# ai4ce/DiscoNet

Measured on AMD Instinct MI355X. Metric: scenes/sec (5-agent 256x256 BEV), higher is better.
Workload: dtype f16 hi+lo pair per value (32 bits; 22-bit significand for |x| >= 0.125, f16 exponent range, lo subnormal below: absolute floor 2^-25); conv products as split-f16 x3 MFMA, f32 accumulate; 1 GPU; DiscoNet det eval forward (--com disco), 5-agent, batch 4 per GPU, 256x256x13 BEV, no KD, sparse voxel lists -> dense -> enc -> DiscoGraph fusion -> dec -> cls/reg heads; agents=5, batch_per_gpu=4, conv_math=sp, launch=hipGraph replay, parallelism=scene-parallel x1 (no data-path collective)

## Files before the change

disconet_amd/csrc/common.hip:

```cpp
#include "dn_internal.h"

namespace dn {
char* err_buf() {
  static thread_local char buf[512] = {0};
  return buf;
}
namespace {
typedef unsigned u32x4 __attribute__((ext_vector_type(4)));
__global__ void __launch_bounds__(256) zero_fill_kernel(unsigned char* p, size_t head, size_t vecs, size_t tail) {
  const size_t tid = blockIdx.x * (size_t)blockDim.x + threadIdx.x, stride = (size_t)gridDim.x * blockDim.x;
  if (tid < head) p[tid] = 0;
  u32x4* v = reinterpret_cast<u32x4*>(p + head);
  for (size_t i = tid; i < vecs; i += stride) v[i] = u32x4{0u, 0u, 0u, 0u};
  if (tid < tail) p[head + 16 * vecs + tid] = 0;
}
}

hipError_t zero_fill(void* ptr, size_t bytes, hipStream_t stream) {
  if (bytes == 0) return hipSuccess;
  unsigned char* p = static_cast<unsigned char*>(ptr);
  size_t head = (16 - (reinterpret_cast<size_t>(p) & 15)) & 15;
  if (head > bytes) head = bytes;
  const size_t vecs = (bytes - head) / 16, tail = bytes - head - 16 * vecs;
  const size_t want = (vecs + 255) / 256;
  const int blocks = (int)(want < 1 ? 1 : (want > 8192 ? 8192 : want));
  hipLaunchKernelGGL(zero_fill_kernel, dim3(blocks), dim3(256), 0, stream, p, head, vecs, tail);
  return hipGetLastError();
}
}

extern "C" int dn_version(void) { return 135; }

#ifndef DN_BUILD_ID
#error "build through disconet_amd/csrc/build.py (it passes -DDN_BUILD_ID)"
#endif
static const char dn_build_id_marker[] = "dn-build-id:" DN_BUILD_ID;
extern "C" const char* dn_build_id(void) { return dn_build_id_marker + 12; }

extern "C" int dn_sp_range_flags_async(unsigned* dst_device, int reset, void* stream) {
  DN_REQUIRE(dst_device != nullptr, "sp_range_flags_async: null destination");
  hipStream_t s = (hipStream_t)stream;
  if ((reset & 2) && dn::zero_fill(dst_device, sizeof(unsigned), s) != hipSuccess)
    return dn::fail(DN_ERR_LAUNCH, "sp_range_flags_async: zero fill of the destination failed");
  const bool clear = (reset & 1) != 0;
  dn::range_collect_conv_sp(dst_device, clear, s);
  dn::range_collect_conv_spq(dst_device, clear, s);
  dn::range_collect_fuse_mlp(dst_device, clear, s);
  dn::range_collect_conv_wgrad(dst_device, clear, s);
  return dn::check_launch("sp_range_collect_kernel");
}

extern "C" unsigned dn_sp_range_flags(int reset) {
  unsigned* d = nullptr;
  unsigned v = 0;
  if (hipDeviceSynchronize() != hipSuccess || hipMalloc((void**)&d, sizeof v) != hipSuccess) return 0x80000000u;
  bool ok = hipMemcpy(d, &v, sizeof v, hipMemcpyHostToDevice) == hipSuccess &&
            dn_sp_range_flags_async(d, reset ? 1 : 0, nullptr) == DN_OK &&
            hipMemcpy(&v, d, sizeof v, hipMemcpyDeviceToHost) == hipSuccess;
  (void)hipFree(d);
  return ok ? v : 0x80000000u;
}

extern "C" const char* dn_last_error(void) { return dn::err_buf(); }
```

disconet_amd/csrc/fuse_mlp.hip:

```cpp
#include "dn_internal.h"
#include "sp_device.h"
#include <type_traits>

#ifndef DN_FUSE_PHASES
#define DN_FUSE_PHASES 0
#endif
#if DN_FUSE_PHASES
__device__ unsigned long long g_fuse_phase[8];
extern "C" int dn_fuse_phase_cycles(unsigned long long* host8, int reset) {
  if (hipDeviceSynchronize() != hipSuccess) return -1;
  if (host8 && hipMemcpyFromSymbol(host8, HIP_SYMBOL(g_fuse_phase), sizeof(unsigned long long) * 8) != hipSuccess) return -1;
  if (reset) { unsigned long long z[8] = {0}; if (hipMemcpyToSymbol(HIP_SYMBOL(g_fuse_phase), z, sizeof z) != hipSuccess) return -1; }
  return 0;
}
#endif

namespace {

constexpr int MAX_AGENTS = 8;
constexpr size_t kW2Bytes = 8 * 2 * 2 * 32 * 16, kW3Bytes = 2 * 2 * 2 * 32 * 16;
constexpr int FUSE_G = 3;
constexpr int FUSE_GL = 2;

struct FuseMlpArgs {
  const float* feat;
  const float* warped;
  const int32_t* num_agent;
  const unsigned char* w1;
  const unsigned char* w2;
  const unsigned char* w3;
  const float *s1, *t1, *s2, *t2, *s3, *t3, *w4, *b4;
  unsigned char* fused_sp;
  float* fused_nhwc;
  float* weights_out;
  int batch, agents, hw, only_v2i, ego_first, ego_count, tiles;
  int total_tiles;
  int warped_fm;
};
constexpr int kWAhead = 1, kWRing = 2;

__device__ inline half8 frag_of(const unsigned char* base, int idx) {
  return *reinterpret_cast<const half8*>(base + (size_t)idx * 16);
}

template <int C, int G, int NW, int WL = 0>
__global__ void __launch_bounds__(64 * (WL > 0 ? WL : NW), (NW == 1 || WL > 0) ? 1 : 2) disco_fuse_mlp_kernel(const FuseMlpArgs a) {
  constexpr bool kWL = WL > 0;
  constexpr int TWV = kWL ? WL : 1;
  static_assert(!kWL || NW == 1, "weight-in-LDS form: one wave per tile");
  constexpr int KS = C / 16;
  constexpr int KSW = KS / NW;
  static_assert(KS % NW == 0, "pass 2 splits the k-steps over the waves");
  constexpr int kW1MatBytes = 4 * KS * 2 * 2 * 32 * 16;
  extern __shared__ __attribute__((aligned(16))) unsigned char w1_s[];
  __shared__ float ek_s[TWV][MAX_AGENTS][64];
  __shared__ float e_s[kWL ? 1 : 64][64];
  __shared__ int jl_s[TWV][MAX_AGENTS];
  __shared__ __attribute__((aligned(16))) unsigned char w23_s[kW2Bytes + kW3Bytes];
  __shared__ __attribute__((aligned(16))) float aff_s[2 * 128 + 2 * 32 + 3 * 8];

  const int lane = threadIdx.x & 63, wave = NW > 1 ? threadIdx.x >> 6 : 0;
  const int tw = kWL ? threadIdx.x >> 6 : 0;
  const int ks_first = wave * KSW;
  const int li = lane & 31, lh = lane >> 5;
  const int wid_raw = kWL ? blockIdx.x * WL + tw : blockIdx.x;
  const bool have = wid_raw < a.total_tiles;
  const int wid = have ? wid_raw : a.total_tiles - 1;
  const int tile = wid % a.tiles, il = (wid / a.tiles) % a.ego_count, b = wid / (a.tiles * a.ego_count);
  const int i = a.ego_first + il;
  const int p = tile * 32 + li;
  const bool pvalid = p < a.hw && have;
  const int pc = p < a.hw ? p : a.hw - 1;
  int live = a.num_agent[b];
  live = live < 0 ? 0 : (live < a.agents ? live : a.agents);
  const size_t oimg = (size_t)il * a.batch + b;

  struct Row {
    const float* p;
    int kss, r1;
  };
  const Row xrow_r = {a.feat + (((size_t)i * a.batch + b) * a.hw + pc) * C + 8 * lh, 16, 4};
  const float* xrow = xrow_r.p;
  auto yrow_of = [&](int j) {
    const int jj = j - (j > i ? 1 : 0);
    const float* pair = a.warped + (((size_t)b * a.ego_count + il) * (a.agents - 1) + jj) * a.hw * C;
    return a.warped_fm ? Row{pair + ((size_t)tile * KS * 2 * 64 + lane) * 4, 512, 256} : Row{pair + (size_t)pc * C + 8 * lh, 16, 4};
  };

  float amax = 0.f;
  bool nan_seen = false;
  auto store_piece = [&](int ks, const f32x4 v0, const f32x4 v1) {
    if (!pvalid) return;
    if (a.fused_sp) {
      u32x2 h0, l0, h1, l1;
      note_nan4(nan_seen, v0);
      note_nan4(nan_seen, v1);
      split4(v0, h0, l0, amax);
      split4(v1, h1, l1, amax);
      const size_t plane = (size_t)a.hw * 16;
      unsigned char* o = a.fused_sp + ((oimg * KS + ks) * 4 + lh) * plane + (size_t)p * 16;
      *reinterpret_cast<u32x4*>(o) = u32x4{h0[0], h0[1], h1[0], h1[1]};
      *reinterpret_cast<u32x4*>(o + 2 * plane) = u32x4{l0[0], l0[1], l1[0], l1[1]};
    }
    if (a.fused_nhwc) {
      float* o = a.fused_nhwc + (oimg * a.hw + p) * C + 16 * ks + 8 * lh;
      *reinterpret_cast<f32x4*>(o) = v0;
      *reinterpret_cast<f32x4*>(o + 4) = v1;
    }
  };

  constexpr int NTHR = 64 * (kWL ? WL : NW);
#if DN_FUSE_PHASES
  unsigned long long ph[8] = {0, 0, 0, 0, 0, 0, 0, 0};
  unsigned long long t_prev = __builtin_readcyclecounter();
  const unsigned long long t_begin = t_prev;
  auto mark = [&](int k) { const unsigned long long t = __builtin_readcyclecounter(); ph[k] += t - t_prev; t_prev = t; };
#else
  auto mark = [&](int) {};
#endif
  if (kWL || i < live) {
    const int t = threadIdx.x;
    for (int q = t; q < (int)((kW2Bytes + kW3Bytes) / 16); q += NTHR)
      *reinterpret_cast<u32x4*>(w23_s + q * 16) = *reinterpret_cast<const u32x4*>(a.w2 + (size_t)q * 16);
    for (int q = t; q < 128; q += NTHR) { aff_s[q] = a.s1[q]; aff_s[128 + q] = a.t1[q]; }
    if (t < 32) { aff_s[256 + t] = a.s2[t]; aff_s[288 + t] = a.t2[t]; }
    if (t < 8) { aff_s[320 + t] = a.s3[t]; aff_s[328 + t] = a.t3[t]; aff_s[336 + t] = a.w4[t]; }
  }
  auto stage_w1 = [&](int mat) {
    if constexpr (kWL) {
      const auto rs = __builtin_amdgcn_make_buffer_rsrc(const_cast<unsigned char*>(a.w1 + (size_t)mat * kW1MatBytes), 0,
                                                        kW1MatBytes, 0x00020000);
      constexpr int INSTR = kW1MatBytes / 1024;
      for (int q = tw; q < INSTR; q += WL) dma16(rs, w1_s + q * 1024, (unsigned)(q * 1024 + lane * 16), 0);
      wait_vm0();
    }
  };
  stage_w1(0);
  const float b4v = a.b4[0];
  const unsigned char* w2l = w23_s;
  const unsigned char* w3l = w23_s + kW2Bytes;
  const float *s1l = aff_s, *t1l = aff_s + 128, *s2l = aff_s + 256, *t2l = aff_s + 288, *s3l = aff_s + 320,
              *t3l = aff_s + 328, *w4l = aff_s + 336;

  const bool active = have && i < live;
  if (i >= live) {
#pragma unroll
    for (int u = 0; u < KSW; ++u) {
      const int ks = ks_first + u;
      store_piece(ks, *reinterpret_cast<const f32x4*>(xrow + 16 * ks),
                  *reinterpret_cast<const f32x4*>(xrow + 16 * ks + 4));
    }
    if constexpr (!kWL) {
      note_range(amax, nan_seen);
      return;
    }
  }

  int n = 1;
  jl_s[tw][0] = i;
  for (int j = 0; j < live; ++j)
    if (j != i && (!a.only_v2i || i == 0 || j == 0)) jl_s[tw][n++] = j;
  if constexpr (NW > 1 || kWL) __syncthreads();
  auto row_of = [&](int k) { return k == 0 ? xrow_r : yrow_of(jl_s[tw][k]); };

  auto frag_from = [&](const f32x4 v0, const f32x4 v1, half8& fh, half8& fl) {
    u32x2 h0, l0, h1, l1;
    split4(v0, h0, l0);
    split4(v1, h1, l1);
    fh = __builtin_bit_cast(half8, u32x4{h0[0], h0[1], h1[0], h1[1]});
    fl = __builtin_bit_cast(half8, u32x4{l0[0], l0[1], l1[0], l1[1]});
  };

  auto layer1 = [&](auto ng_c, const Row (&rows)[G], int cnt, int mat, f32x16 (&acc)[G][4]) {
    constexpr int NG = decltype(ng_c)::value;
    const unsigned char* wbase = a.w1 + (size_t)mat * 4 * KS * 2 * 2 * 32 * 16 + (size_t)(lh * 32 + li) * 16;
    half8 wh[kWRing][4], wl[kWRing][4];
    constexpr int RING = 4;
    f32x4 r0[RING][NG], r1[RING][NG];
    auto wload = [&](int ks, int s) {
#pragma unroll
      for (int nt = 0; nt < 4; ++nt) {
        if constexpr (kWL) {
          wh[s][nt] = *reinterpret_cast<const half8*>(w1_s + (((nt * KS + ks) * 2 + 0) * 64 + lh * 32 + li) * 16);
          wl[s][nt] = *reinterpret_cast<const half8*>(w1_s + (((nt * KS + ks) * 2 + 1) * 64 + lh * 32 + li) * 16);
        } else {
          wh[s][nt] = *reinterpret_cast<const half8*>(wbase + (size_t)(((nt * KS + ks) * 2 + 0) * 64) * 16);
          wl[s][nt] = *reinterpret_cast<const half8*>(wbase + (size_t)(((nt * KS + ks) * 2 + 1) * 64) * 16);
        }
      }
    };
    auto rload = [&](int ks, int s) {
#pragma unroll
      for (int g = 0; g < NG; ++g)
        if (g < cnt) {
          r0[s][g] = *reinterpret_cast<const f32x4*>(rows[g].p + ks * rows[g].kss);
          r1[s][g] = *reinterpret_cast<const f32x4*>(rows[g].p + ks * rows[g].kss + rows[g].r1);
        }
    };
    auto mma = [&](int sw, int sr) {
#pragma unroll
      for (int g = 0; g < NG; ++g)
        if (g < cnt) {
          half8 fh, fl;
          frag_from(r0[sr][g], r1[sr][g], fh, fl);
#pragma unroll
          for (int nt = 0; nt < 4; ++nt) acc[g][nt] = __builtin_amdgcn_mfma_f32_32x32x16_f16(wl[sw][nt], fh, acc[g][nt], 0, 0, 0);
#pragma unroll
          for (int nt = 0; nt < 4; ++nt) acc[g][nt] = __builtin_amdgcn_mfma_f32_32x32x16_f16(wh[sw][nt], fl, acc[g][nt], 0, 0, 0);
#pragma unroll
          for (int nt = 0; nt < 4; ++nt) acc[g][nt] = __builtin_amdgcn_mfma_f32_32x32x16_f16(wh[sw][nt], fh, acc[g][nt], 0, 0, 0);
        }
    };
    static_assert(KS % RING == 0, "k loop runs RING k-steps per trip");
#pragma unroll
    for (int q = 0; q < RING - 1; ++q) rload(q, q);
#pragma unroll
    for (int q = 0; q < kWAhead; ++q) wload(q, q);
#pragma unroll 1
    for (int ks0 = 0; ks0 < KS; ks0 += RING) {
#pragma unroll
      for (int u = 0; u < RING; ++u) {
        const int ks = ks0 + u;
        if (ks + RING - 1 < KS) rload(ks + RING - 1, (u + RING - 1) % RING);
        if (ks + kWAhead < KS) wload(ks + kWAhead, (u + kWAhead) & (kWRing - 1));
        __builtin_amdgcn_sched_barrier(0);
        mma(u & (kWRing - 1), u);
        __builtin_amdgcn_sched_barrier(0);
      }
    }
  };

  auto tail = [&](f32x16 (&acc)[4]) -> float {
    f32x16 acc2;
#pragma unroll
    for (int r = 0; r < 16; ++r) acc2[r] = 0.f;
#pragma unroll
    for (int nt = 0; nt < 4; ++nt) {
      u32x2 hi[4], lo[4];
#pragma unroll
      for (int g = 0; g < 4; ++g) {
        const int u = nt * 32 + 8 * g + 4 * lh;
        const f32x4 sc = *reinterpret_cast<const f32x4*>(s1l + u), sh = *reinterpret_cast<const f32x4*>(t1l + u);
        float unused = 0.f;
        split4(affine4(quad_of(acc[nt], g), sc, sh), hi[g], lo[g], unused, 0.f);
      }
#pragma unroll
      for (int m = 0; m < 2; ++m) {
        const int ks = nt * 2 + m;
        const half8 xh = __builtin_bit_cast(half8, gather_octet(hi[2 * m], hi[2 * m + 1]));
        const half8 xl = __builtin_bit_cast(half8, gather_octet(lo[2 * m], lo[2 * m + 1]));
        const half8 wh = frag_of(w2l, ((ks * 2 + 0) * 2 + lh) * 32 + li), wl = frag_of(w2l, ((ks * 2 + 1) * 2 + lh) * 32 + li);
        acc2 = __builtin_amdgcn_mfma_f32_32x32x16_f16(wl, xh, acc2, 0, 0, 0);
        acc2 = __builtin_amdgcn_mfma_f32_32x32x16_f16(wh, xl, acc2, 0, 0, 0);
        acc2 = __builtin_amdgcn_mfma_f32_32x32x16_f16(wh, xh, acc2, 0, 0, 0);
      }
    }
    f32x16 acc3;
#pragma unroll
    for (int r = 0; r < 16; ++r) acc3[r] = 0.f;
    {
      u32x2 hi[4], lo[4];
#pragma unroll
      for (int g = 0; g < 4; ++g) {
        const int u = 8 * g + 4 * lh;
        const f32x4 sc = *reinterpret_cast<const f32x4*>(s2l + u), sh = *reinterpret_cast<const f32x4*>(t2l + u);
        float unused = 0.f;
        split4(affine4(quad_of(acc2, g), sc, sh), hi[g], lo[g], unused, 0.f);
      }
#pragma unroll
      for (int m = 0; m < 2; ++m) {
        const half8 xh = __builtin_bit_cast(half8, gather_octet(hi[2 * m], hi[2 * m + 1]));
        const half8 xl = __builtin_bit_cast(half8, gather_octet(lo[2 * m], lo[2 * m + 1]));
        const half8 wh = frag_of(w3l, ((m * 2 + 0) * 2 + lh) * 32 + li), wl = frag_of(w3l, ((m * 2 + 1) * 2 + lh) * 32 + li);
        acc3 = __builtin_amdgcn_mfma_f32_32x32x16_f16(wl, xh, acc3, 0, 0, 0);
        acc3 = __builtin_amdgcn_mfma_f32_32x32x16_f16(wh, xl, acc3, 0, 0, 0);
        acc3 = __builtin_amdgcn_mfma_f32_32x32x16_f16(wh, xh, acc3, 0, 0, 0);
      }
    }
    const f32x4 sc = *reinterpret_cast<const f32x4*>(s3l + 4 * lh), sh = *reinterpret_cast<const f32x4*>(t3l + 4 * lh);
    const f32x4 w4 = *reinterpret_cast<const f32x4*>(w4l + 4 * lh);
    float part = 0.f;
#pragma unroll
    for (int e = 0; e < 4; ++e) part += fmaxf(acc3[e] * sc[e] + sh[e], 0.f) * w4[e];
    const float other = __shfl_xor(part, 32, 64);
    const float s = fmaxf((lh ? other + part : part + other) + b4v, 0.f);
    return expf(s);
  };

  f32x16 Ereg[kWL ? 4 : 1];
  mark(0);
  if constexpr (kWL) {
    if (active) {
      f32x16 acc[G][4];
#pragma unroll
      for (int nt = 0; nt < 4; ++nt)
#pragma unroll
        for (int r = 0; r < 16; ++r) acc[0][nt][r] = 0.f;
      Row rows[G];
#pragma unroll
      for (int g = 0; g < G; ++g) rows[g] = xrow_r;
      layer1(std::integral_constant<int, 1>{}, rows, 1, 0, acc);
#pragma unroll
      for (int nt = 0; nt < 4; ++nt) Ereg[nt] = acc[0][nt];
#if DN_FUSE_PHASES
      { float probe = Ereg[0][0]; asm volatile("v_mov_b32 %0, %0" : "+v"(probe)); }
#endif
    }
    mark(1);
    __syncthreads();
    stage_w1(1);
    __syncthreads();
    mark(0);
  } else if constexpr (NW == 1) {
    f32x16 acc[G][4];
#pragma unroll
    for (int nt = 0; nt < 4; ++nt)
#pragma unroll
      for (int r = 0; r < 16; ++r) acc[0][nt][r] = 0.f;
    Row rows[G];
#pragma unroll
    for (int g = 0; g < G; ++g) rows[g] = xrow_r;
    layer1(std::integral_constant<int, 1>{}, rows, 1, 0, acc);
#pragma unroll
    for (int nt = 0; nt < 4; ++nt)
#pragma unroll
      for (int r = 0; r < 16; ++r) e_s[nt * 16 + r][lane] = acc[0][nt][r];
  } else {
    static_assert(NW == 1 || NW == 4, "one layer-1 unit tile per wave");
    f32x16 acc;
#pragma unroll
    for (int r = 0; r < 16; ++r) acc[r] = 0.f;
    const unsigned char* wb = a.w1 + (size_t)(lh * 32 + li) * 16 + (size_t)(wave * KS) * 2 * 64 * 16;
    half8 wh[2], wl[2];
    f32x4 r0[4], r1[4];
    auto wload = [&](int ks, int sl) {
      wh[sl] = *reinterpret_cast<const half8*>(wb + (size_t)((ks * 2 + 0) * 64) * 16);
      wl[sl] = *reinterpret_cast<const half8*>(wb + (size_t)((ks * 2 + 1) * 64) * 16);
    };
    auto rload = [&](int ks, int sl) {
      r0[sl] = *reinterpret_cast<const f32x4*>(xrow + 16 * ks);
      r1[sl] = *reinterpret_cast<const f32x4*>(xrow + 16 * ks + 4);
    };
    rload(0, 0);
    rload(1, 1);
    rload(2, 2);
    wload(0, 0);
#pragma unroll 1
    for (int ks0 = 0; ks0 < KS; ks0 += 4) {
#pragma unroll
      for (int u = 0; u < 4; ++u) {
        const int ks = ks0 + u;
        if (ks + 3 < KS) rload(ks + 3, (u + 3) & 3);
        if (ks + 1 < KS) wload(ks + 1, (u + 1) & 1);
        half8 fh, fl;
        frag_from(r0[u], r1[u], fh, fl);
        acc = __builtin_amdgcn_mfma_f32_32x32x16_f16(wl[u & 1], fh, acc, 0, 0, 0);
        acc = __builtin_amdgcn_mfma_f32_32x32x16_f16(wh[u & 1], fl, acc, 0, 0, 0);
        acc = __builtin_amdgcn_mfma_f32_32x32x16_f16(wh[u & 1], fh, acc, 0, 0, 0);
      }
    }
#pragma unroll
    for (int r = 0; r < 16; ++r) e_s[wave * 16 + r][lane] = acc[r];
    __syncthreads();
  }
  if constexpr (kWL) {
    if (!active) {
      note_range(amax, nan_seen);
      return;
    }
  }
  if constexpr (NW == 1) {
    for (int g0 = 0; g0 < n; g0 += G) {
      const int cnt = n - g0 < G ? n - g0 : G;
      f32x16 acc[G][4];
      Row rows[G];
#pragma unroll
      for (int g = 0; g < G; ++g) {
        rows[g] = row_of(g0 + g < n ? g0 + g : 0);
        if (g < cnt) {
#pragma unroll
          for (int nt = 0; nt < 4; ++nt) {
            if constexpr (kWL) acc[g][nt] = Ereg[nt];
            else {
#pragma unroll
              for (int r = 0; r < 16; ++r) acc[g][nt][r] = e_s[nt * 16 + r][lane];
            }
          }
        }
      }
      layer1(std::integral_constant<int, G>{}, rows, cnt, 1, acc);
#if DN_FUSE_PHASES
      { float probe = acc[0][0][0]; asm volatile("v_mov_b32 %0, %0" : "+v"(probe)); }
#endif
      mark(2);
#pragma unroll
      for (int g = 0; g < G; ++g)
        if (g < cnt) ek_s[tw][g0 + g][lane] = tail(acc[g]);
      mark(3);
    }
  } else {
    for (int k = wave; k < n; k += NW) {
      f32x16 acc[G][4];
      Row rows[G];
#pragma unroll
      for (int g = 0; g < G; ++g) rows[g] = row_of(k);
#pragma unroll
      for (int nt = 0; nt < 4; ++nt)
#pragma unroll
        for (int r = 0; r < 16; ++r) acc[0][nt][r] = e_s[nt * 16 + r][lane];
      layer1(std::integral_constant<int, 1>{}, rows, 1, 1, acc);
      ek_s[0][k][lane] = tail(acc[0]);
    }
    __syncthreads();
  }
  float den = 0.f;
  for (int k = 0; k < n; ++k) den += ek_s[tw][k][lane];

  f32x4 f0[KSW], f1[KSW], y0[2][KSW], y1[2][KSW];
  auto yload = [&](int k, int s) {
    const Row row = row_of(k);
#pragma unroll
    for (int ks = 0; ks < KSW; ++ks) {
      y0[s][ks] = *reinterpret_cast<const f32x4*>(row.p + (ks_first + ks) * row.kss);
      y1[s][ks] = *reinterpret_cast<const f32x4*>(row.p + (ks_first + ks) * row.kss + row.r1);
    }
  };
  auto yacc = [&](int k, int s) {
    const float w = ek_s[tw][k][lane] / den;
    if (a.weights_out && pvalid && lh == 0 && wave == 0)
      a.weights_out[(((size_t)b * a.ego_count + il) * a.agents + k) * a.hw + p] = w;
#pragma unroll
    for (int ks = 0; ks < KSW; ++ks) {
      f0[ks] += y0[s][ks] * w;
      f1[ks] += y1[s][ks] * w;
    }
  };
#pragma unroll
  for (int ks = 0; ks < KSW; ++ks) f0[ks] = f1[ks] = f32x4{0.f, 0.f, 0.f, 0.f};
  yload(0, 0);
  for (int k = 0; k < n; k += 2) {
    if (k + 1 < n) yload(k + 1, 1);
    yacc(k, 0);
    if (k + 1 < n) {
      if (k + 2 < n) yload(k + 2, 0);
      yacc(k + 1, 1);
    }
  }
#pragma unroll
  for (int ks = 0; ks < KSW; ++ks) store_piece(ks_first + ks, f0[ks], f1[ks]);
  note_range(amax, nan_seen);
#if DN_FUSE_PHASES
  mark(4);
  ph[5] = 1;
  ph[6] = __builtin_readcyclecounter() - t_begin;
  if (lane == 0)
    for (int k = 0; k < 7; ++k) atomicAdd(&g_fuse_phase[k], ph[k]);
#endif
}

__global__ void pack_frags_kernel(const float* __restrict__ w, int ld, int col0, int rows, int cols,
                                  int n_tiles, int ksteps, float wmul, unsigned char* __restrict__ out) {
  const int idx = blockIdx.x * blockDim.x + threadIdx.x;
  if (idx >= n_tiles * ksteps * 2 * 32) return;
  const int row = idx % 32, h = (idx / 32) % 2, ks = (idx / 64) % ksteps, nt = idx / (64 * ksteps);
  half8 hi, lo;
#pragma unroll
  for (int e = 0; e < 8; ++e) {
    const int r = nt * 32 + row, c = ks * 16 + h * 8 + e;
    float v = (r < rows && c < cols) ? w[(size_t)r * ld + col0 + c] * wmul : 0.f;
    v = fminf(fmaxf(v, -65504.f), 65504.f);
    hi[e] = (_Float16)v;
    lo[e] = (_Float16)(v - (float)hi[e]);
  }
  *reinterpret_cast<half8*>(out + (size_t)((((nt * ksteps + ks) * 2 + 0) * 2 + h) * 32 + row) * 16) = hi;
  *reinterpret_cast<half8*>(out + (size_t)((((nt * ksteps + ks) * 2 + 1) * 2 + h) * 32 + row) * 16) = lo;
}

inline size_t w1_bytes(int c) { return (size_t)2 * 4 * (c / 16) * 2 * 2 * 32 * 16; }

}

namespace dn { void range_collect_fuse_mlp(unsigned* dst, bool reset, hipStream_t s) { sp_range_collect_here(dst, reset, s); } }

int g_fuse_waves = 0;

extern "C" int dn_fuse_mlp_set_waves(int waves) {
  DN_REQUIRE(waves == 0 || waves == 1 || waves == 2 || waves == 4,
             "fuse_mlp: form is 1 or 4 waves per tile, 2 = layer-1 weights in LDS (0 = default), got %d", waves);
  g_fuse_waves = waves;
  return DN_OK;
}

extern "C" int dn_fuse_mlp_supported(int c) { return c == 64 || c == 128 || c == 256; }

extern "C" size_t dn_fuse_mlp_packed_bytes(int c) { return w1_bytes(c) + kW2Bytes + kW3Bytes; }

extern "C" int dn_fuse_mlp_pack(const float* w1, const float* w2, const float* w3, int c, float wmul1,
                                float wmul2, float wmul3, void* packed, void* stream) {
  DN_REQUIRE(w1 && w2 && w3 && packed, "fuse_mlp pack: null pointer");
  DN_REQUIRE(dn_fuse_mlp_supported(c), "fuse_mlp pack: %d channels unsupported (64, 128 or 256)", c);
  hipStream_t s = (hipStream_t)stream;
  unsigned char* out = (unsigned char*)packed;
  const int ks = c / 16;
  for (int mat = 0; mat < 2; ++mat)
    hipLaunchKernelGGL(pack_frags_kernel, dim3((4 * ks * 64 + 255) / 256), dim3(256), 0, s, w1, 2 * c, mat * c,
                       128, c, 4, ks, wmul1, out + (size_t)mat * (w1_bytes(c) / 2));
  hipLaunchKernelGGL(pack_frags_kernel, dim3((8 * 64 + 255) / 256), dim3(256), 0, s, w2, 128, 0, 32, 128, 1, 8,
                     wmul2, out + w1_bytes(c));
  hipLaunchKernelGGL(pack_frags_kernel, dim3((2 * 64 + 255) / 256), dim3(256), 0, s, w3, 32, 0, 8, 32, 1, 2,
                     wmul3, out + w1_bytes(c) + kW2Bytes);
  return dn::check_launch("pack_frags_kernel");
}

namespace {
template <int CC, int WL>
int launch_wl(const FuseMlpArgs& a, dim3 grid, int lds, hipStream_t s) {
  auto kern = disco_fuse_mlp_kernel<CC, FUSE_GL, 1, WL>;
  static dn::PerDeviceFlag flag;
  bool& done = flag.here();
  if (!done) {
    if (hipFuncSetAttribute(reinterpret_cast<const void*>(kern), hipFuncAttributeMaxDynamicSharedMemorySize, lds) != hipSuccess)
      return dn::fail(DN_ERR_LAUNCH, "fuse_mlp: cannot reserve %d B of dynamic LDS", lds);
    done = true;
  }
  hipLaunchKernelGGL(kern, grid, dim3(64 * WL), lds, s, a);
  return dn::check_launch("disco_fuse_mlp_kernel (weights in LDS)");
}

int fuse_mlp_impl(const float* feat, const float* warped, int warped_fm, const int32_t* num_agent, const dn_fuse_mlp_params* p,
                  int batch, int agents, int hw, int c, int only_v2i, int ego_first, int ego_count, void* fused_sp,
                  float* fused_nhwc, float* weights_out, void* stream);
}

extern "C" int dn_disco_fuse_mlp(const float* feat, const float* warped, const int32_t* num_agent,
                                 const dn_fuse_mlp_params* p, int batch, int agents, int hw, int c,
                                 int only_v2i, int ego_first, int ego_count, void* fused_sp,
                                 float* fused_nhwc, float* weights_out, void* stream) {
  return fuse_mlp_impl(feat, warped, 0, num_agent, p, batch, agents, hw, c, only_v2i, ego_first, ego_count, fused_sp,
                       fused_nhwc, weights_out, stream);
}

extern "C" int dn_disco_fuse_mlp_fm(const float* feat, const float* warped_fm, const int32_t* num_agent,
                                    const dn_fuse_mlp_params* p, int batch, int agents, int hw, int c,
                                    int only_v2i, int ego_first, int ego_count, void* fused_sp,
                                    float* fused_nhwc, float* weights_out, void* stream) {
  DN_REQUIRE(hw % 32 == 0, "fuse_mlp (fragment-major): hw %d must be a multiple of 32", hw);
  return fuse_mlp_impl(feat, warped_fm, 1, num_agent, p, batch, agents, hw, c, only_v2i, ego_first, ego_count, fused_sp,
                       fused_nhwc, weights_out, stream);
}

namespace {
int fuse_mlp_impl(const float* feat, const float* warped, int warped_fm, const int32_t* num_agent, const dn_fuse_mlp_params* p,
                  int batch, int agents, int hw, int c, int only_v2i, int ego_first, int ego_count, void* fused_sp,
                  float* fused_nhwc, float* weights_out, void* stream) {
  DN_REQUIRE(feat && num_agent && p && (fused_sp || fused_nhwc), "fuse_mlp: null pointer");
  DN_REQUIRE(agents < 2 || warped, "fuse_mlp: neighbours present but warped is null");
  DN_REQUIRE(batch > 0 && agents > 0 && hw > 0, "fuse_mlp: empty problem");
  DN_REQUIRE(dn_fuse_mlp_supported(c), "fuse_mlp: %d channels unsupported (64, 128 or 256)", c);
  DN_REQUIRE(ego_first >= 0 && ego_count > 0 && ego_first + ego_count <= agents,
             "fuse_mlp: ego range [%d, %d) outside 0..%d", ego_first, ego_first + ego_count, agents);
  DN_REQUIRE(agents <= MAX_AGENTS, "fuse_mlp: at most %d agents supported (got %d)", MAX_AGENTS, agents);
  DN_REQUIRE(p->packed && p->s1 && p->t1 && p->s2 && p->t2 && p->s3 && p->t3 && p->w4 && p->b4,
             "fuse_mlp: null MLP parameter");
  auto aligned16 = [](const void* q) { return (reinterpret_cast<uintptr_t>(q) & 15) == 0; };
  DN_REQUIRE(aligned16(feat) && aligned16(warped) && aligned16(p->packed) && aligned16(fused_sp) &&
                 aligned16(fused_nhwc) && aligned16(p->s1) && aligned16(p->t1) && aligned16(p->s2) &&
                 aligned16(p->t2) && aligned16(p->s3) && aligned16(p->t3) && aligned16(p->w4),
             "fuse_mlp: buffers must be 16-byte aligned");
  FuseMlpArgs a;
  a.feat = feat; a.warped = warped; a.num_agent = num_agent;
  a.w1 = (const unsigned char*)p->packed;
  a.w2 = a.w1 + w1_bytes(c);
  a.w3 = a.w2 + kW2Bytes;
  a.s1 = p->s1; a.t1 = p->t1; a.s2 = p->s2; a.t2 = p->t2; a.s3 = p->s3; a.t3 = p->t3; a.w4 = p->w4; a.b4 = p->b4;
  a.fused_sp = (unsigned char*)fused_sp; a.fused_nhwc = fused_nhwc; a.weights_out = weights_out;
  a.batch = batch; a.agents = agents; a.hw = hw; a.only_v2i = only_v2i;
  a.ego_first = ego_first; a.ego_count = ego_count;
  a.tiles = (hw + 31) / 32;
  a.total_tiles = batch * ego_count * a.tiles;
  a.warped_fm = warped_fm;
  dim3 grid(a.total_tiles);
  hipStream_t s = (hipStream_t)stream;
  const int waves = g_fuse_waves > 0 ? g_fuse_waves : (grid.x < 2u * 256u ? 4 : 2);
  if (waves == 2) {
    const int wl = a.total_tiles <= 2 * 256 ? 2 : a.total_tiles <= 3 * 256 ? 3 : 4;
    const dim3 g2((a.total_tiles + wl - 1) / wl);
    const int lds = 4 * (c / 16) * 2 * 2 * 32 * 16;
    int rc = DN_OK;
#define DN_FUSE_WL(CC)                                                                        \
    rc = wl == 2 ? launch_wl<CC, 2>(a, g2, lds, s) : wl == 3 ? launch_wl<CC, 3>(a, g2, lds, s) : launch_wl<CC, 4>(a, g2, lds, s)
    if (c == 256) DN_FUSE_WL(256);
    else if (c == 128) DN_FUSE_WL(128);
    else DN_FUSE_WL(64);
#undef DN_FUSE_WL
    if (rc) return rc;
  } else if (waves == 1) {
    if (c == 256) hipLaunchKernelGGL((disco_fuse_mlp_kernel<256, FUSE_G, 1>), grid, dim3(64), 0, s, a);
    else if (c == 128) hipLaunchKernelGGL((disco_fuse_mlp_kernel<128, FUSE_G, 1>), grid, dim3(64), 0, s, a);
    else hipLaunchKernelGGL((disco_fuse_mlp_kernel<64, FUSE_G, 1>), grid, dim3(64), 0, s, a);
  } else {
    if (c == 256) hipLaunchKernelGGL((disco_fuse_mlp_kernel<256, 1, 4>), grid, dim3(256), 0, s, a);
    else if (c == 128) hipLaunchKernelGGL((disco_fuse_mlp_kernel<128, 1, 4>), grid, dim3(256), 0, s, a);
    else hipLaunchKernelGGL((disco_fuse_mlp_kernel<64, 1, 4>), grid, dim3(256), 0, s, a);
  }
  return dn::check_launch("disco_fuse_mlp_kernel");
}
}
```

Measured before the change: 2299 scenes/s.

## Add persistent unit-split fusion MLP kernel splitting channels across four waves

Adds a new persistent form of the DiscoGraph fusion MLP kernel for 256 channels. Each of four waves owns a quarter of the channel k-steps and keeps its slice of the neighbour layer-1 weights in registers. Converted input fragments are shared through a double-buffered LDS slot, and per-wave partial layer-1 sums are exchanged through LDS so the small MLP tail runs once per agent on one wave. It becomes the default when there are many tiles and C is 256, aiming to cut repeated weight loading and raise MFMA utilisation. The cost is more block-wide barriers and LDS traffic per agent.

```diff
diff --git a/disconet_amd/csrc/common.hip b/disconet_amd/csrc/common.hip
--- a/disconet_amd/csrc/common.hip
+++ b/disconet_amd/csrc/common.hip
@@ -29,7 +29,7 @@
 }
 }
 
-extern "C" int dn_version(void) { return 135; }
+extern "C" int dn_version(void) { return 136; }
 
 #ifndef DN_BUILD_ID
 #error "build through disconet_amd/csrc/build.py (it passes -DDN_BUILD_ID)"
diff --git a/disconet_amd/csrc/fuse_mlp.hip b/disconet_amd/csrc/fuse_mlp.hip
--- a/disconet_amd/csrc/fuse_mlp.hip
+++ b/disconet_amd/csrc/fuse_mlp.hip
@@ -43,6 +43,104 @@
   return *reinterpret_cast<const half8*>(base + (size_t)idx * 16);
 }
 
+
+__device__ inline void frag_from(const f32x4 v0, const f32x4 v1, half8& fh, half8& fl) {
+  u32x2 h0, l0, h1, l1;
+  split4(v0, h0, l0);
+  split4(v1, h1, l1);
+  fh = __builtin_bit_cast(half8, u32x4{h0[0], h0[1], h1[0], h1[1]});
+  fl = __builtin_bit_cast(half8, u32x4{l0[0], l0[1], l1[0], l1[1]});
+}
+
+template <int KS>
+__device__ inline void store_piece_of(const FuseMlpArgs& a, bool pvalid, size_t oimg, int p, int lh, int ks, const f32x4 v0,
+                                      const f32x4 v1, float& amax, bool& nan_seen) {
+  if (!pvalid) return;
+  if (a.fused_sp) {
+    u32x2 h0, l0, h1, l1;
+    note_nan4(nan_seen, v0);
+    note_nan4(nan_seen, v1);
+    split4(v0, h0, l0, amax);
+    split4(v1, h1, l1, amax);
+    const size_t plane = (size_t)a.hw * 16;
+    unsigned char* o = a.fused_sp + ((oimg * KS + ks) * 4 + lh) * plane + (size_t)p * 16;
+    *reinterpret_cast<u32x4*>(o) = u32x4{h0[0], h0[1], h1[0], h1[1]};
+    *reinterpret_cast<u32x4*>(o + 2 * plane) = u32x4{l0[0], l0[1], l1[0], l1[1]};
+  }
+  if (a.fused_nhwc) {
+    float* o = a.fused_nhwc + (oimg * a.hw + p) * (KS * 16) + 16 * ks + 8 * lh;
+    *reinterpret_cast<f32x4*>(o) = v0;
+    *reinterpret_cast<f32x4*>(o + 4) = v1;
+  }
+}
+
+struct MlpTail {
+  const unsigned char *w2l, *w3l;
+  const float *s1l, *t1l, *s2l, *t2l, *s3l, *t3l, *w4l;
+  float b4v;
+  int li, lh;
+};
+__device__ inline float mlp_tail(const MlpTail& t, f32x16 (&acc)[4]) {
+  const unsigned char *w2l = t.w2l, *w3l = t.w3l;
+  const float *s1l = t.s1l, *t1l = t.t1l, *s2l = t.s2l, *t2l = t.t2l, *s3l = t.s3l, *t3l = t.t3l, *w4l = t.w4l;
+  const float b4v = t.b4v;
+  const int li = t.li, lh = t.lh;
+  f32x16 acc2;
+#pragma unroll
+  for (int r = 0; r < 16; ++r) acc2[r] = 0.f;
+#pragma unroll
+  for (int nt = 0; nt < 4; ++nt) {
+    u32x2 hi[4], lo[4];
+#pragma unroll
+    for (int g = 0; g < 4; ++g) {
+      const int u = nt * 32 + 8 * g + 4 * lh;
+      const f32x4 sc = *reinterpret_cast<const f32x4*>(s1l + u), sh = *reinterpret_cast<const f32x4*>(t1l + u);
+      float unused = 0.f;
+      split4(affine4(quad_of(acc[nt], g), sc, sh), hi[g], lo[g], unused, 0.f);
+    }
+#pragma unroll
+    for (int m = 0; m < 2; ++m) {
+      const int ks = nt * 2 + m;
+      const half8 xh = __builtin_bit_cast(half8, gather_octet(hi[2 * m], hi[2 * m + 1]));
+      const half8 xl = __builtin_bit_cast(half8, gather_octet(lo[2 * m], lo[2 * m + 1]));
+      const half8 wh = frag_of(w2l, ((ks * 2 + 0) * 2 + lh) * 32 + li), wl = frag_of(w2l, ((ks * 2 + 1) * 2 + lh) * 32 + li);
+      acc2 = __builtin_amdgcn_mfma_f32_32x32x16_f16(wl, xh, acc2, 0, 0, 0);
+      acc2 = __builtin_amdgcn_mfma_f32_32x32x16_f16(wh, xl, acc2, 0, 0, 0);
+      acc2 = __builtin_amdgcn_mfma_f32_32x32x16_f16(wh, xh, acc2, 0, 0, 0);
+    }
+  }
+  f32x16 acc3;
+#pragma unroll
+  for (int r = 0; r < 16; ++r) acc3[r] = 0.f;
+  {
+    u32x2 hi[4], lo[4];
+#pragma unroll
+    for (int g = 0; g < 4; ++g) {
+      const int u = 8 * g + 4 * lh;
+      const f32x4 sc = *reinterpret_cast<const f32x4*>(s2l + u), sh = *reinterpret_cast<const f32x4*>(t2l + u);
+      float unused = 0.f;
+      split4(affine4(quad_of(acc2, g), sc, sh), hi[g], lo[g], unused, 0.f);
+    }
+#pragma unroll
+    for (int m = 0; m < 2; ++m) {
+      const half8 xh = __builtin_bit_cast(half8, gather_octet(hi[2 * m], hi[2 * m + 1]));
+      const half8 xl = __builtin_bit_cast(half8, gather_octet(lo[2 * m], lo[2 * m + 1]));
+      const half8 wh = frag_of(w3l, ((m * 2 + 0) * 2 + lh) * 32 + li), wl = frag_of(w3l, ((m * 2 + 1) * 2 + lh) * 32 + li);
+      acc3 = __builtin_amdgcn_mfma_f32_32x32x16_f16(wl, xh, acc3, 0, 0, 0);
+      acc3 = __builtin_amdgcn_mfma_f32_32x32x16_f16(wh, xl, acc3, 0, 0, 0);
+      acc3 = __builtin_amdgcn_mfma_f32_32x32x16_f16(wh, xh, acc3, 0, 0, 0);
+    }
+  }
+  const f32x4 sc = *reinterpret_cast<const f32x4*>(s3l + 4 * lh), sh = *reinterpret_cast<const f32x4*>(t3l + 4 * lh);
+  const f32x4 w4 = *reinterpret_cast<const f32x4*>(w4l + 4 * lh);
+  float part = 0.f;
+#pragma unroll
+  for (int e = 0; e < 4; ++e) part += fmaxf(acc3[e] * sc[e] + sh[e], 0.f) * w4[e];
+  const float other = __shfl_xor(part, 32, 64);
+  const float s = fmaxf((lh ? other + part : part + other) + b4v, 0.f);
+  return expf(s);
+}
+
 template <int C, int G, int NW, int WL = 0>
 __global__ void __launch_bounds__(64 * (WL > 0 ? WL : NW), (NW == 1 || WL > 0) ? 1 : 2) disco_fuse_mlp_kernel(const FuseMlpArgs a) {
   constexpr bool kWL = WL > 0;
@@ -90,23 +188,7 @@
   float amax = 0.f;
   bool nan_seen = false;
   auto store_piece = [&](int ks, const f32x4 v0, const f32x4 v1) {
-    if (!pvalid) return;
-    if (a.fused_sp) {
-      u32x2 h0, l0, h1, l1;
-      note_nan4(nan_seen, v0);
-      note_nan4(nan_seen, v1);
-      split4(v0, h0, l0, amax);
-      split4(v1, h1, l1, amax);
-      const size_t plane = (size_t)a.hw * 16;
-      unsigned char* o = a.fused_sp + ((oimg * KS + ks) * 4 + lh) * plane + (size_t)p * 16;
-      *reinterpret_cast<u32x4*>(o) = u32x4{h0[0], h0[1], h1[0], h1[1]};
-      *reinterpret_cast<u32x4*>(o + 2 * plane) = u32x4{l0[0], l0[1], l1[0], l1[1]};
-    }
-    if (a.fused_nhwc) {
-      float* o = a.fused_nhwc + (oimg * a.hw + p) * C + 16 * ks + 8 * lh;
-      *reinterpret_cast<f32x4*>(o) = v0;
-      *reinterpret_cast<f32x4*>(o + 4) = v1;
-    }
+    store_piece_of<KS>(a, pvalid, oimg, p, lh, ks, v0, v1, amax, nan_seen);
   };
 
   constexpr int NTHR = 64 * (kWL ? WL : NW);
@@ -163,14 +245,6 @@
   if constexpr (NW > 1 || kWL) __syncthreads();
   auto row_of = [&](int k) { return k == 0 ? xrow_r : yrow_of(jl_s[tw][k]); };
 
-  auto frag_from = [&](const f32x4 v0, const f32x4 v1, half8& fh, half8& fl) {
-    u32x2 h0, l0, h1, l1;
-    split4(v0, h0, l0);
-    split4(v1, h1, l1);
-    fh = __builtin_bit_cast(half8, u32x4{h0[0], h0[1], h1[0], h1[1]});
-    fl = __builtin_bit_cast(half8, u32x4{l0[0], l0[1], l1[0], l1[1]});
-  };
-
   auto layer1 = [&](auto ng_c, const Row (&rows)[G], int cnt, int mat, f32x16 (&acc)[G][4]) {
     constexpr int NG = decltype(ng_c)::value;
     const unsigned char* wbase = a.w1 + (size_t)mat * 4 * KS * 2 * 2 * 32 * 16 + (size_t)(lh * 32 + li) * 16;
@@ -230,62 +304,8 @@
     }
   };
 
-  auto tail = [&](f32x16 (&acc)[4]) -> float {
-    f32x16 acc2;
-#pragma unroll
-    for (int r = 0; r < 16; ++r) acc2[r] = 0.f;
-#pragma unroll
-    for (int nt = 0; nt < 4; ++nt) {
-      u32x2 hi[4], lo[4];
-#pragma unroll
-      for (int g = 0; g < 4; ++g) {
-        const int u = nt * 32 + 8 * g + 4 * lh;
-        const f32x4 sc = *reinterpret_cast<const f32x4*>(s1l + u), sh = *reinterpret_cast<const f32x4*>(t1l + u);
-        float unused = 0.f;
-        split4(affine4(quad_of(acc[nt], g), sc, sh), hi[g], lo[g], unused, 0.f);
-      }
-#pragma unroll
-      for (int m = 0; m < 2; ++m) {
-        const int ks = nt * 2 + m;
-        const half8 xh = __builtin_bit_cast(half8, gather_octet(hi[2 * m], hi[2 * m + 1]));
-        const half8 xl = __builtin_bit_cast(half8, gather_octet(lo[2 * m], lo[2 * m + 1]));
-        const half8 wh = frag_of(w2l, ((ks * 2 + 0) * 2 + lh) * 32 + li), wl = frag_of(w2l, ((ks * 2 + 1) * 2 + lh) * 32 + li);
-        acc2 = __builtin_amdgcn_mfma_f32_32x32x16_f16(wl, xh, acc2, 0, 0, 0);
-        acc2 = __builtin_amdgcn_mfma_f32_32x32x16_f16(wh, xl, acc2, 0, 0, 0);
-        acc2 = __builtin_amdgcn_mfma_f32_32x32x16_f16(wh, xh, acc2, 0, 0, 0);
-      }
-    }
-    f32x16 acc3;
-#pragma unroll
-    for (int r = 0; r < 16; ++r) acc3[r] = 0.f;
-    {
-      u32x2 hi[4], lo[4];
-#pragma unroll
-      for (int g = 0; g < 4; ++g) {
-        const int u = 8 * g + 4 * lh;
-        const f32x4 sc = *reinterpret_cast<const f32x4*>(s2l + u), sh = *reinterpret_cast<const f32x4*>(t2l + u);
-        float unused = 0.f;
-        split4(affine4(quad_of(acc2, g), sc, sh), hi[g], lo[g], unused, 0.f);
-      }
-#pragma unroll
-      for (int m = 0; m < 2; ++m) {
-        const half8 xh = __builtin_bit_cast(half8, gather_octet(hi[2 * m], hi[2 * m + 1]));
-        const half8 xl = __builtin_bit_cast(half8, gather_octet(lo[2 * m], lo[2 * m + 1]));
-        const half8 wh = frag_of(w3l, ((m * 2 + 0) * 2 + lh) * 32 + li), wl = frag_of(w3l, ((m * 2 + 1) * 2 + lh) * 32 + li);
-        acc3 = __builtin_amdgcn_mfma_f32_32x32x16_f16(wl, xh, acc3, 0, 0, 0);
-        acc3 = __builtin_amdgcn_mfma_f32_32x32x16_f16(wh, xl, acc3, 0, 0, 0);
-        acc3 = __builtin_amdgcn_mfma_f32_32x32x16_f16(wh, xh, acc3, 0, 0, 0);
-      }
-    }
-    const f32x4 sc = *reinterpret_cast<const f32x4*>(s3l + 4 * lh), sh = *reinterpret_cast<const f32x4*>(t3l + 4 * lh);
-    const f32x4 w4 = *reinterpret_cast<const f32x4*>(w4l + 4 * lh);
-    float part = 0.f;
-#pragma unroll
-    for (int e = 0; e < 4; ++e) part += fmaxf(acc3[e] * sc[e] + sh[e], 0.f) * w4[e];
-    const float other = __shfl_xor(part, 32, 64);
-    const float s = fmaxf((lh ? other + part : part + other) + b4v, 0.f);
-    return expf(s);
-  };
+  const MlpTail tt = {w2l, w3l, s1l, t1l, s2l, t2l, s3l, t3l, w4l, b4v, li, lh};
+  auto tail = [&](f32x16 (&acc)[4]) -> float { return mlp_tail(tt, acc); };
 
   f32x16 Ereg[kWL ? 4 : 1];
   mark(0);
@@ -458,6 +478,261 @@
 #endif
 }
 
+template <int R_>
+struct UnitSplit {
+  static constexpr int R = R_;
+};
+template <int... I, class F>
+__device__ __forceinline__ void static_for(std::integer_sequence<int, I...>, F&& f) {
+  (f(std::integral_constant<int, I>{}), ...);
+}
+
+template <class Form, int C>
+__global__ void __launch_bounds__(256, 1) disco_fuse_mlp_kernel(const FuseMlpArgs a) {
+  constexpr int R = Form::R;
+  constexpr int KS = C / 16, KQ = KS / 4;
+  static_assert(KS % 4 == 0, "a channel quarter is a whole number of k-steps");
+  static_assert(R >= 0 && R <= MAX_AGENTS, "retained slots");
+  constexpr int kW1MatBytes = 4 * KS * 2 * 2 * 32 * 16;
+  constexpr int kFragSlot = KS * 2 * 64 * 16;
+  constexpr int kXchSlot = 4 * 4 * 64 * 16;
+  extern __shared__ __attribute__((aligned(16))) unsigned char us_s[];
+  __shared__ float ek_s[MAX_AGENTS][64];
+  __shared__ int jl_s[MAX_AGENTS];
+  __shared__ __attribute__((aligned(16))) unsigned char w23_s[kW2Bytes + kW3Bytes];
+  __shared__ __attribute__((aligned(16))) float aff_s[2 * 128 + 2 * 32 + 3 * 8];
+  unsigned char* const frag_s = us_s;
+  unsigned char* const xch_s = us_s + 2 * kFragSlot;
+
+  const int lane = threadIdx.x & 63, wave = threadIdx.x >> 6;
+  const int li = lane & 31, lh = lane >> 5;
+  const int ks_first = wave * KQ;
+#if DN_FUSE_PHASES
+  unsigned long long ph[8] = {0, 0, 0, 0, 0, 0, 0, 0};
+  unsigned long long t_prev = __builtin_readcyclecounter();
+  const unsigned long long t_begin = t_prev;
+  auto mark = [&](int k) { const unsigned long long t = __builtin_readcyclecounter(); ph[k] += t - t_prev; t_prev = t; };
+#else
+  auto mark = [&](int) {};
+#endif
+  {
+    const int t = threadIdx.x;
+    for (int q = t; q < (int)((kW2Bytes + kW3Bytes) / 16); q += 256)
+      *reinterpret_cast<u32x4*>(w23_s + q * 16) = *reinterpret_cast<const u32x4*>(a.w2 + (size_t)q * 16);
+    if (t < 128) { aff_s[t] = a.s1[t]; aff_s[128 + t] = a.t1[t]; }
+    if (t < 32) { aff_s[256 + t] = a.s2[t]; aff_s[288 + t] = a.t2[t]; }
+    if (t < 8) { aff_s[320 + t] = a.s3[t]; aff_s[328 + t] = a.t3[t]; aff_s[336 + t] = a.w4[t]; }
+  }
+  const unsigned char* const w_ego = a.w1 + ((size_t)(wave * KS) * 2 * 64 + lane) * 16;
+  const unsigned char* const w_nbr = w_ego + kW1MatBytes;
+  half8 wh[KS], wl[KS];
+#pragma unroll
+  for (int ks = 0; ks < KS; ++ks) {
+    wh[ks] = frag_of(w_nbr, (ks * 2 + 0) * 64);
+    wl[ks] = frag_of(w_nbr, (ks * 2 + 1) * 64);
+  }
+  const MlpTail tt = {w23_s, w23_s + kW2Bytes, aff_s, aff_s + 128, aff_s + 256, aff_s + 288, aff_s + 320, aff_s + 328, aff_s + 336,
+                      a.b4[0], li, lh};
+  float amax = 0.f;
+  bool nan_seen = false;
+  __syncthreads();
+
+  for (int wid = blockIdx.x; wid < a.total_tiles; wid += gridDim.x) {
+    const int tile = wid % a.tiles, il = (wid / a.tiles) % a.ego_count, b = wid / (a.tiles * a.ego_count);
+    const int i = a.ego_first + il;
+    const int p = tile * 32 + li;
+    const bool pvalid = p < a.hw;
+    const int pc = pvalid ? p : a.hw - 1;
+    int live = a.num_agent[b];
+    live = live < 0 ? 0 : (live < a.agents ? live : a.agents);
+    const size_t oimg = (size_t)il * a.batch + b;
+    struct Row {
+      const float* p;
+      int kss, r1;
+    };
+    const Row xrow_r = {a.feat + (((size_t)i * a.batch + b) * a.hw + pc) * C + 8 * lh, 16, 4};
+    auto store_piece = [&](int ks, const f32x4 v0, const f32x4 v1) {
+      store_piece_of<KS>(a, pvalid, oimg, p, lh, ks, v0, v1, amax, nan_seen);
+    };
+    if (i >= live) {
+#pragma unroll
+      for (int u = 0; u < KQ; ++u) {
+        const int ks = ks_first + u;
+        store_piece(ks, *reinterpret_cast<const f32x4*>(xrow_r.p + 16 * ks), *reinterpret_cast<const f32x4*>(xrow_r.p + 16 * ks + 4));
+      }
+      continue;
+    }
+    constexpr int kEgoRing = KS < 4 ? KS : 4;
+    half8 eh[kEgoRing], el[kEgoRing];
+#pragma unroll
+    for (int q = 0; q < kEgoRing; ++q) {
+      eh[q] = frag_of(w_ego, (q * 2 + 0) * 64);
+      el[q] = frag_of(w_ego, (q * 2 + 1) * 64);
+    }
+    __syncthreads();
+    int n = 1;
+    jl_s[0] = i;
+    for (int j = 0; j < live; ++j)
+      if (j != i && (!a.only_v2i || i == 0 || j == 0)) jl_s[n++] = j;
+    auto row_of = [&](int k) {
+      if (k == 0) return xrow_r;
+      const int j = jl_s[k];
+      const int jj = j - (j > i ? 1 : 0);
+      const float* pair = a.warped + (((size_t)b * a.ego_count + il) * (a.agents - 1) + jj) * a.hw * C;
+      return a.warped_fm ? Row{pair + ((size_t)tile * KS * 2 * 64 + lane) * 4, 512, 256} : Row{pair + (size_t)pc * C + 8 * lh, 16, 4};
+    };
+
+    f32x4 y0[R > 0 ? R : 1][KQ], y1[R > 0 ? R : 1][KQ];
+    f32x4 z0[KQ], z1[KQ];
+    auto rload = [&](auto kc) {
+      constexpr int k = decltype(kc)::value;
+      const Row row = row_of(k);
+#pragma unroll
+      for (int u = 0; u < KQ; ++u) {
+        const f32x4 v0 = *reinterpret_cast<const f32x4*>(row.p + (ks_first + u) * row.kss);
+        const f32x4 v1 = *reinterpret_cast<const f32x4*>(row.p + (ks_first + u) * row.kss + row.r1);
+        if constexpr (k < R) { y0[k][u] = v0; y1[k][u] = v1; }
+        else { z0[u] = v0; z1[u] = v1; }
+      }
+    };
+    auto fwrite = [&](auto kc) {
+      constexpr int k = decltype(kc)::value;
+      unsigned char* fb = frag_s + (k & 1) * kFragSlot + lane * 16;
+#pragma unroll
+      for (int u = 0; u < KQ; ++u) {
+        half8 fh, fl;
+        if constexpr (k < R) frag_from(y0[k][u], y1[k][u], fh, fl);
+        else frag_from(z0[u], z1[u], fh, fl);
+        *reinterpret_cast<half8*>(fb + ((ks_first + u) * 2 + 0) * 1024) = fh;
+        *reinterpret_cast<half8*>(fb + ((ks_first + u) * 2 + 1) * 1024) = fl;
+      }
+    };
+    rload(std::integral_constant<int, 0>{});
+    fwrite(std::integral_constant<int, 0>{});
+    __syncthreads();
+    mark(0);
+
+    f32x16 E;
+    half8 fh[2], fl[2];
+    auto fread = [&](const unsigned char* fb, int ks, int sl) {
+      fh[sl] = *reinterpret_cast<const half8*>(fb + (ks * 2 + 0) * 1024);
+      fl[sl] = *reinterpret_cast<const half8*>(fb + (ks * 2 + 1) * 1024);
+    };
+    static_for(std::make_integer_sequence<int, MAX_AGENTS / 4>{}, [&](auto gc) {
+      constexpr int g = decltype(gc)::value;
+      static_for(std::make_integer_sequence<int, 4>{}, [&](auto sc) {
+        constexpr int k = 4 * g + decltype(sc)::value;
+        if (k < n) {
+          auto next_rows = [&] {
+            if constexpr (k + 1 < MAX_AGENTS) {
+              if (k + 1 < n) rload(std::integral_constant<int, k + 1>{});
+            }
+          };
+          if constexpr (k > 0) next_rows();
+          const unsigned char* fb = frag_s + (k & 1) * kFragSlot + lane * 16;
+          if constexpr (k == 0) {
+#pragma unroll
+            for (int r = 0; r < 16; ++r) E[r] = 0.f;
+            fread(fb, 0, 0);
+#pragma unroll
+            for (int ks = 0; ks < KS; ++ks) {
+              if (ks + 1 < KS) fread(fb, ks + 1, (ks + 1) & 1);
+              __builtin_amdgcn_sched_barrier(0);
+              E = __builtin_amdgcn_mfma_f32_32x32x16_f16(el[ks % kEgoRing], fh[ks & 1], E, 0, 0, 0);
+              E = __builtin_amdgcn_mfma_f32_32x32x16_f16(eh[ks % kEgoRing], fl[ks & 1], E, 0, 0, 0);
+              E = __builtin_amdgcn_mfma_f32_32x32x16_f16(eh[ks % kEgoRing], fh[ks & 1], E, 0, 0, 0);
+              if (ks + kEgoRing < KS) {
+                eh[ks % kEgoRing] = frag_of(w_ego, ((ks + kEgoRing) * 2 + 0) * 64);
+                el[ks % kEgoRing] = frag_of(w_ego, ((ks + kEgoRing) * 2 + 1) * 64);
+              }
+              __builtin_amdgcn_sched_barrier(0);
+            }
+#if DN_FUSE_PHASES
+            { float probe = E[0]; asm volatile("v_mov_b32 %0, %0" : "+v"(probe)); }
+#endif
+            mark(1);
+            next_rows();
+          }
+          f32x16 acc = E;
+          fread(fb, 0, 0);
+#pragma unroll
+          for (int ks = 0; ks < KS; ++ks) {
+            if (ks + 1 < KS) fread(fb, ks + 1, (ks + 1) & 1);
+            __builtin_amdgcn_sched_barrier(0);
+            acc = __builtin_amdgcn_mfma_f32_32x32x16_f16(wl[ks], fh[ks & 1], acc, 0, 0, 0);
+            acc = __builtin_amdgcn_mfma_f32_32x32x16_f16(wh[ks], fl[ks & 1], acc, 0, 0, 0);
+            acc = __builtin_amdgcn_mfma_f32_32x32x16_f16(wh[ks], fh[ks & 1], acc, 0, 0, 0);
+            __builtin_amdgcn_sched_barrier(0);
+          }
+          unsigned char* xb = xch_s + (k & 3) * kXchSlot + (wave * 4 * 64 + lane) * 16;
+#pragma unroll
+          for (int q = 0; q < 4; ++q) *reinterpret_cast<f32x4*>(xb + q * 1024) = quad_of(acc, q);
+          mark(2);
+          if constexpr (k + 1 < MAX_AGENTS) {
+            if (k + 1 < n) fwrite(std::integral_constant<int, k + 1>{});
+          }
+          __syncthreads();
+          mark(0);
+        }
+      });
+      if (4 * g < n) {
+        const int s = 4 * g + wave;
+        if (s < n) {
+          f32x16 acc4[4];
+          const unsigned char* xb = xch_s + (s & 3) * kXchSlot + lane * 16;
+#pragma unroll
+          for (int nt = 0; nt < 4; ++nt)
+#pragma unroll
+            for (int q = 0; q < 4; ++q) {
+              const f32x4 v = *reinterpret_cast<const f32x4*>(xb + (nt * 4 + q) * 1024);
+#pragma unroll
+              for (int e = 0; e < 4; ++e) acc4[nt][4 * q + e] = v[e];
+            }
+          ek_s[s][lane] = mlp_tail(tt, acc4);
+        }
+        mark(3);
+        __syncthreads();
+        mark(0);
+      }
+    });
+
+    float den = 0.f;
+    for (int k = 0; k < n; ++k) den += ek_s[k][lane];
+    f32x4 f0[KQ], f1[KQ];
+#pragma unroll
+    for (int u = 0; u < KQ; ++u) f0[u] = f1[u] = f32x4{0.f, 0.f, 0.f, 0.f};
+    static_for(std::make_integer_sequence<int, MAX_AGENTS>{}, [&](auto kc) {
+      constexpr int k = decltype(kc)::value;
+      if (k < n) {
+        if constexpr (k >= R) rload(kc);
+        const float w = ek_s[k][lane] / den;
+        if (a.weights_out && pvalid && lh == 0 && wave == 0)
+          a.weights_out[(((size_t)b * a.ego_count + il) * a.agents + k) * a.hw + p] = w;
+#pragma unroll
+        for (int u = 0; u < KQ; ++u) {
+          if constexpr (k < R) {
+            f0[u] += y0[k][u] * w;
+            f1[u] += y1[k][u] * w;
+          } else {
+            f0[u] += z0[u] * w;
+            f1[u] += z1[u] * w;
+          }
+        }
+      }
+    });
+#pragma unroll
+    for (int u = 0; u < KQ; ++u) store_piece(ks_first + u, f0[u], f1[u]);
+    mark(4);
+  }
+  note_range(amax, nan_seen);
+#if DN_FUSE_PHASES
+  ph[5] = 1;
+  ph[6] = __builtin_readcyclecounter() - t_begin;
+  if (lane == 0)
+    for (int k = 0; k < 7; ++k) atomicAdd(&g_fuse_phase[k], ph[k]);
+#endif
+}
+
 __global__ void pack_frags_kernel(const float* __restrict__ w, int ld, int col0, int rows, int cols,
                                   int n_tiles, int ksteps, float wmul, unsigned char* __restrict__ out) {
   const int idx = blockIdx.x * blockDim.x + threadIdx.x;
@@ -485,8 +760,8 @@
 int g_fuse_waves = 0;
 
 extern "C" int dn_fuse_mlp_set_waves(int waves) {
-  DN_REQUIRE(waves == 0 || waves == 1 || waves == 2 || waves == 4,
-             "fuse_mlp: form is 1 or 4 waves per tile, 2 = layer-1 weights in LDS (0 = default), got %d", waves);
+  DN_REQUIRE(waves >= 0 && waves <= 4,
+             "fuse_mlp: form is 1 or 4 waves per tile, 2 = layer-1 weights in LDS, 3 = unit-split (0 = default), got %d", waves);
   g_fuse_waves = waves;
   return DN_OK;
 }
@@ -525,6 +800,22 @@
   }
   hipLaunchKernelGGL(kern, grid, dim3(64 * WL), lds, s, a);
   return dn::check_launch("disco_fuse_mlp_kernel (weights in LDS)");
+}
+
+constexpr int FUSE_US_R = 5;
+template <int CC>
+int launch_us(const FuseMlpArgs& a, hipStream_t s) {
+  auto kern = disco_fuse_mlp_kernel<UnitSplit<FUSE_US_R>, CC>;
+  constexpr int lds = 2 * (CC / 16) * 2 * 64 * 16 + 4 * (4 * 4 * 64 * 16);
+  static dn::PerDeviceFlag flag;
+  bool& done = flag.here();
+  if (!done) {
+    if (hipFuncSetAttribute(reinterpret_cast<const void*>(kern), hipFuncAttributeMaxDynamicSharedMemorySize, lds) != hipSuccess)
+      return dn::fail(DN_ERR_LAUNCH, "fuse_mlp: cannot reserve %d B of dynamic LDS", lds);
+    done = true;
+  }
+  hipLaunchKernelGGL(kern, dim3(a.total_tiles < 256 ? a.total_tiles : 256), dim3(256), lds, s, a);
+  return dn::check_launch("disco_fuse_mlp_kernel (unit-split)");
 }
 
 int fuse_mlp_impl(const float* feat, const float* warped, int warped_fm, const int32_t* num_agent, const dn_fuse_mlp_params* p,
@@ -581,8 +872,11 @@
   a.warped_fm = warped_fm;
   dim3 grid(a.total_tiles);
   hipStream_t s = (hipStream_t)stream;
-  const int waves = g_fuse_waves > 0 ? g_fuse_waves : (grid.x < 2u * 256u ? 4 : 2);
-  if (waves == 2) {
+  DN_REQUIRE(g_fuse_waves != 3 || c == 256, "fuse_mlp: the unit-split form (3) is built for 256 channels, got %d", c);
+  const int waves = g_fuse_waves > 0 ? g_fuse_waves : (grid.x < 2u * 256u ? 4 : c == 256 ? 3 : 2);
+  if (waves == 3) {
+    if (int rc = launch_us<256>(a, s)) return rc;
+  } else if (waves == 2) {
     const int wl = a.total_tiles <= 2 * 256 ? 2 : a.total_tiles <= 3 * 256 ? 3 : 4;
     const dim3 g2((a.total_tiles + wl - 1) / wl);
     const int lds = 4 * (c / 16) * 2 * 2 * 32 * 16;
```

Result: no change. 2312 scenes/s, median of 6 (+0.6%).
